# real-world-cryprography/APSU

Measured on AMD Instinct MI355X. Metric: sender query-eval ms (ComputePowers + all BinBundles + gather), 16M-4096 params, lower is better.
Workload: dtype u64; 1 GPU; 16M-4096: n=8192, 4 bundle indices x 7 BinBundles (degrees [1303, 170]), 6 source -> 72 target powers, ps_low_degree=44; db_bytes_rank0=5459379072, binbundles_rank0=28, parallelism=binbundle-shard x1

## Files before the change

apsu_amd/csrc/c_api.cpp:

```cpp
#include "../../include/apsu_he.h"

#include <algorithm>
#include <thread>
#include <atomic>
#include <cstdlib>
#include <cstring>
#include <new>
#include <string>

#include "db_file.h"
#include "engine.h"
#include "multi.h"
#include "wire.h"
#include "seal_codec.h"

using namespace apsu_he;

#include <condition_variable>
#include <mutex>
#include <unordered_set>

struct apsu_he_powers;
struct apsu_he_ctx { std::unique_ptr<Engine> eng; std::unordered_set<apsu_he_powers *> live_powers; int recycling = 0; };
struct apsu_he_relin { std::unique_ptr<RelinKeys> rk; };
// ... 33 lines not shown
        return APSU_HE_OK;
    } catch (const std::invalid_argument &e) { g_last_error = e.what(); return APSU_HE_INVALID_ARGUMENT;
    } catch (const std::logic_error &e) { g_last_error = e.what(); return APSU_HE_LOGIC_ERROR;
    } catch (const std::bad_alloc &e) { g_last_error = e.what(); return APSU_HE_OUT_OF_MEMORY;
    } catch (const HipError &e) {
        g_last_error = e.what();
        if (g_last_error.find("no HIP device") != std::string::npos) return APSU_HE_NO_DEVICE;
        if (g_last_error.find("out of memory") != std::string::npos) return APSU_HE_OUT_OF_MEMORY;
        return APSU_HE_RUNTIME_ERROR;
    } catch (const std::exception &e) { g_last_error = e.what(); return APSU_HE_RUNTIME_ERROR;
    } catch (...) { g_last_error = "unknown error"; return APSU_HE_RUNTIME_ERROR; }
}

#define REQUIRE(cond, msg) do { if (!(cond)) throw std::invalid_argument(msg); } while (0)

extern "C" {

const char *apsu_he_last_error(void) { return g_last_error.c_str(); }
int apsu_he_abi_version(void) { return APSU_HE_ABI_VERSION; }

int apsu_he_create(const char *json, int device, apsu_he_ctx **out)
{
    return guarded([&] {
        REQUIRE(json && out, "null argument");
        PSUParams p = PSUParams::Load(json);
        HeParams hp = HeParams::FromPSUParams(p);
        auto c = new apsu_he_ctx;
        try { c->eng = std::make_unique<Engine>(hp, &p, device); } catch (...) { delete c; throw; }
        *out = c;
    });
}

int apsu_he_create_raw(uint64_t n, const uint64_t *coeff_modulus, int k, uint64_t plain_modulus, int device, apsu_he_ctx **out)
{
    return guarded([&] {
        REQUIRE(coeff_modulus && out && k > 0, "null argument");
        for (int j = 0; j < k; j++) REQUIRE(!(coeff_modulus[j] >> 60), "coeff_modulus prime has more than 60 bits");
        HeParams hp = HeParams::Create((size_t)n, std::vector<u64>(coeff_modulus, coeff_modulus + k), plain_modulus);
        auto c = new apsu_he_ctx;
        try { c->eng = std::make_unique<Engine>(hp, nullptr, device); } catch (...) { delete c; throw; }
        *out = c;
    });
}

int apsu_he_destroy(apsu_he_ctx *ctx)
{
    return guarded([&] {
        if (!ctx) return;
        {
            std::unique_lock<std::mutex> g(g_registry_mu);
            g_registry_cv.wait(g, [&] { return ctx->recycling == 0; });
            for (apsu_he_powers *p : ctx->live_powers) { p->ctx = nullptr; p->p.reset(); }
            ctx->live_powers.clear();
// ... 320 lines not shown
int apsu_he_compute_powers_cost(const apsu_he_ctx *ctx, uint64_t *cost)
{
    return guarded([&] {
        REQUIRE(ctx && cost, "null argument");
        REQUIRE(ctx->eng->psu(), "context was created without PSUParams");
        const PowersDag &dag = ctx->eng->dag();
        *cost = 110u * (uint64_t)(dag.target_powers().size() - dag.source_count());
    });
}

int apsu_he_multi_create(const char *json, const int *devices, int n_devices, apsu_he_multi **out)
{
    return guarded([&] {
        REQUIRE(json && devices && out && n_devices > 0, "null argument");
        PSUParams p = PSUParams::Load(json);
        HeParams hp = HeParams::FromPSUParams(p);
        auto m = new apsu_he_multi;
        try { m->m = std::make_unique<MultiEngine>(hp, p, std::vector<int>(devices, devices + n_devices)); } catch (...) { delete m; throw; }
        *out = m;
    });
}
int apsu_he_multi_destroy(apsu_he_multi *m) { return guarded([&] { delete m; }); }
int apsu_he_multi_device_count(const apsu_he_multi *m, int *n_devices)
{ return guarded([&] { REQUIRE(m && n_devices, "null argument"); *n_devices = m->m->device_count(); }); }
int apsu_he_multi_result_polys(const apsu_he_multi *m, uint32_t *polys)
{ return guarded([&] { REQUIRE(m && polys, "null argument"); *polys = m->m->engine(0).result_polys(); }); }
int apsu_he_multi_relin_upload(apsu_he_multi *m, const uint64_t *ksk)
{ return guarded([&] { REQUIRE(m && ksk, "null argument"); m->m->upload_relin_keys(ksk); }); }
int apsu_he_multi_db_upload_bundle(apsu_he_multi *m, int device_slot, uint32_t bundle_idx, uint32_t cache_idx, uint32_t n_coeffs,
                                   const uint64_t *const *coeff_ptrs, const uint8_t *is_ntt, int *bundle_id)
{
// ... 889 lines not shown
```

apsu_amd/csrc/engine.cpp:

```cpp
#include "engine.h"
#include "sched_policy.h"
#include "seal_codec.h"

#include <algorithm>
#include <array>
#include <cstdlib>
#include <cstring>
#include <stdexcept>

namespace apsu_he {
static uint32_t packed_row_bits(u64 q);

void throw_hip(hipError_t e, const char *file, int line)
{
    throw HipError(std::string("HIP error: ") + hipGetErrorString(e) + " at " + file + ":" + std::to_string(line));
}
#define HIP_CHECK(x) do { hipError_t e_ = (x); if (e_ != hipSuccess) throw_hip(e_, __FILE__, __LINE__); } while (0)

namespace { struct ArenaOverflow { size_t need; }; }

struct Engine::Enter {
    std::lock_guard<std::mutex> lock;
    int prev = -1;
    explicit Enter(Engine *e) : lock(e->mu_)
// ... 104 lines not shown
        }
        d_tabs_.alloc(tabs.size() * sizeof(NttTable));
        HIP_CHECK(hipMemcpy(d_tabs_.p(), tabs.data(), tabs.size() * sizeof(NttTable), hipMemcpyHostToDevice));
        if (const char *v = std::getenv("APSU_HE_SPLIT")) two_stream_default_ = std::atoi(v) != 0 ? 1 : 0;
        if (split_ntt) fuse_tensor_ = false;
        if (const char *v = std::getenv("APSU_HE_MAC_KARA")) mac_kara_ = std::atoi(v) != 0 ? 1 : 0;
        if (const char *v = std::getenv("APSU_HE_EVAL_SIDE")) eval_side_ = std::atoi(v) != 0;
        if (const char *v = std::getenv("APSU_HE_PACKED_ROWS")) packed_rows_ = std::atoi(v) != 0;
        if (!hp_.using_keyswitching) packed_rows_ = false;
        if (const char *v = std::getenv("APSU_HE_EVAL_WS_BYTES")) eval_ws_budget_ = std::strtoull(v, nullptr, 10);
        if (const char *v = std::getenv("APSU_HE_EVAL_PER_TERM")) force_per_term_ = std::atoi(v) != 0;
        if (const char *v = std::getenv("APSU_HE_SEED_EXPAND_HOST")) seed_expand_host_ = std::atoi(v) != 0;
        ntt_latency_limbs_ = NTT_FORM_AUTO;
        data_primes_narrow_ = true;
        for (int j = 0; j < hp_.K; j++) data_primes_narrow_ = data_primes_narrow_ && ntt_is_narrow(hp_.key_q[j], hp_.logn);
        if (const char *v = std::getenv("APSU_HE_FUSE_TAIL")) fuse_tail_ = std::atoi(v) != 0;
        if (const char *v = std::getenv("APSU_HE_NTT_LATENCY_LIMBS")) ntt_latency_limbs_ = std::strtoull(v, nullptr, 10);
    }
    {
        const int nl = hp_.first_chain_idx + 1;
        std::vector<DevLevel> lv(nl);
        std::vector<int> map_ext((size_t)nl * DMAXE, 0), map_ks((size_t)nl * (DMAXL + 1) * DMAXL, 0),
            map_ksacc((size_t)nl * (DMAXL + 1), 0);
        const u64 mt = (u64)1 << 32;
        for (int c = 0; c < nl; c++) {
            const LevelConstants &h = hp_.level[c];
            DevLevel &d = lv[c];
            std::memset(&d, 0, sizeof(d));
            const int L = h.L, nB = h.nB, nBsk = nB + 1;
            if (L > DMAXL || nBsk > DMAXB) throw std::invalid_argument("too many RNS limbs");
// ... 834 lines not shown
    Enter g(this);
    TIER1_SLOTS();
    check_level(chain_idx);
    check_tier1_residues(a, 2, chain_idx, "multiply: operand holds a coefficient outside [0, q)");
    if (b != a) check_tier1_residues(b, 2, chain_idx, "multiply: operand holds a coefficient outside [0, q)");
    const size_t n = hp_.n, L = chain_idx + 1;
    const int E = hlevel(chain_idx).L + hlevel(chain_idx).nB + 1;
    const bool square = (a == b);
    WITH_ARENA({
        const int nop = square ? 1 : 2;
        u64 *in = ws((size_t)nop * 2 * L * n);
        H2D(in, a, 2 * L * n);
        if (!square) H2D(in + 2 * L * n, b, 2 * L * n);
        u64 *ext = ws((size_t)nop * 2 * E * n);
        { PROF(P_BEHZ_EXT, 0); launch_behz_ext(dlevel(chain_idx), hlevel(chain_idx).L, hlevel(chain_idx).nB, in, L * n, 1, ext, n, nop * 2, st_); }
        d_ntt(ext, (size_t)nop * 2 * E, map_ext(chain_idx), E, false, false);
        u64 *d = ws((size_t)3 * E * n), *o = ws(3 * L * n);
        std::vector<TensorJob> tj{ TensorJob{ ext, square ? ext : ext + (size_t)2 * E * n, d } };
        { PROF(P_TENSOR, 0); launch_tensor(dlevel(chain_idx), upload_jobs(tj), n, 1, st_); }
        d_ntt(d, (size_t)3 * E, map_ext_fin(chain_idx), E, true, false);
        std::vector<FinishJob> fj{ FinishJob{ d, o, 1, 0 } };
        { PROF(P_BEHZ_FINISH, 0); launch_behz_finish(dlevel(chain_idx), hlevel(chain_idx).L, hlevel(chain_idx).nB, upload_jobs(fj), false, n, 1, st_); }
        D2H(out3, o, 3 * L * n);
        tier1_done();
    });
}

void Engine::relinearize(u64 *ct3, const RelinKeys &rk, int chain_idx)
{
    Enter g(this);
    TIER1_SLOTS();
    check_level(chain_idx);
    check_tier1_residues(ct3, 3, chain_idx, "relinearize: operand holds a coefficient outside [0, q)");
    if (!hp_.using_keyswitching) throw std::logic_error("parameters do not support key switching");
    const size_t n = hp_.n, L = chain_idx + 1;
// ... 292 lines not shown
                run.dbuf = ws(max_nodes * nb * 3 * Ef * n);
            }
            run.arena_mark = arena_off_;
            return;
        }
        if (stage > 0) {
            if ((size_t)stage >= s.levels.size()) return;
            u64 *dbuf = run.dbuf;
            {
                const size_t d = (size_t)stage;
                arena_off_ = run.arena_mark;
                const auto &pl = s.levels[d - 1];
                const int npar = pl.sp - pl.s0;
                if (npar > 0) {
                    if (run.ext_done != (int)d - 1) { PROFW(P_BEHZ_EXT, (size_t)npar * nb * 2 * n * (Lf + Ef)); launch_behz_ext(dlevel(first), hlevel(first).L, hlevel(first).nB, slot_ptr(pl.s0, 0), slot_w, 2, ext_ptr(pl.s0, 0), n, npar * nb, st_); }
                    d_ntt(ext_ptr(pl.s0, 0), (size_t)npar * nb * 2 * Ef, map_ext(first), (int)Ef, false, false);
                }
                const auto &cl = s.levels[d];
                const int nn = cl.s1 - cl.s0;
                if (nn <= 0) return;
                std::vector<TensorJob> tj;
                std::vector<FinishJob> fj;
                for (auto &nd : s.nodes) {
                    if (nd[0] < cl.s0 || nd[0] >= cl.s1) continue;
                    for (int b = 0; b < nb; b++) {
                        u64 *dd = dbuf + ((size_t)(nd[0] - cl.s0) * nb + b) * 3 * Ef * n;
                        tj.push_back(TensorJob{ ext_ptr(nd[1], b), ext_ptr(nd[2], b), dd });
                        fj.push_back(FinishJob{ dd, slot_ptr(nd[0], b), 1, 0 });
                    }
                }
                if (fuse_tensor_) {
                    PROF(P_NTT_FUSED, tj.size() * 3 * Ef);
                    launch_intt_tensor(hp_.logn, upload_jobs(tj), (int)tj.size(), (int)Ef, Ef * n, nullptr, 0, tabs(), map_ext_fin(first), (int)Ef, st_, ntt_latency_limbs_);
                } else {
                    { PROF(P_TENSOR, 0); launch_tensor(dlevel(first), upload_jobs(tj), n, (int)tj.size(), st_); }
                    d_ntt(dbuf, (size_t)nn * nb * 3 * Ef, map_ext_fin(first), (int)Ef, true, false);
                }
                { PROFW(P_BEHZ_FINISH, fj.size() * 3 * n * (Ef + Lf)); launch_behz_finish(dlevel(first), hlevel(first).L, hlevel(first).nB, upload_jobs(fj), false, n, (int)fj.size(), st_); }
                if (hp_.using_keyswitching && nn > 0) {
                    const int npar_here = ((size_t)d + 1 < s.levels.size()) ? (cl.sp - cl.s0) : 0;
                    if (d_relinearize(slot_ptr(cl.s0, 0), slot_w, nn * nb, *rk, first, npar_here ? ext_ptr(cl.s0, 0) : nullptr, npar_here * nb))
                        run.ext_done = (int)d;
                }
            }
            return;
        }
        arena_off_ = run.arena_mark;
        auto convert = [&](const std::vector<uint32_t> &powers, int target, u64 *out) {
            if (powers.empty()) return;
            const int cnt = (int)powers.size() * nb;
            std::vector<CtJob> jobs;
// ... 28 lines not shown
            for (int b = 0; b < nb; b++)
                for (size_t i = 0; i < np; i++)
                    for (size_t pl = 0; pl < 2 * Lf; pl++)
                        srcp[(((size_t)b * np + i) * 2 * Lf) + pl] = slot_ptr(s.slot_of[s.low_powers[i]], b) + pl * n;
            bool nored = hp_.logn <= 14;
            for (size_t j = 0; j < Lf && nored; j++) nored = ntt_gather_nored_ok(hp_.key_q[j], hp_.key_q[j], hp_.logn);
            PROF(P_NTT_FWD, srcp.size());
            launch_ntt_gather(hp_.logn, upload_jobs(srcp), pw->low.u(), srcp.size(), tabs(), map_ct(), (int)Lf, st_, nored, ntt_latency_limbs_, data_primes_narrow_);
        } else if (do_low) {
            convert(s.low_powers, low_target, pw->low.u());
            d_ntt_ct(pw->low.u(), (size_t)pw->n_low * nb * 2, low_target, false);
        }
        if (do_high && pw->n_high) {
            convert(s.high_powers, high, pw->high.u());
            { PROFW(P_BEHZ_EXT, (size_t)pw->n_high * nb * 2 * n * (Lh + Eh)); launch_behz_ext(dlevel(high), hlevel(high).L, hlevel(high).nB, pw->high.u(), Lh * n, 1, pw->hext.u(), n, (int)(pw->n_high * nb * 2), st_); }
            d_ntt(pw->hext.u(), (size_t)pw->n_high * nb * 2 * Eh, map_ext(high), (int)Eh, false, false);
        }
    }
}

std::unique_ptr<Powers> Engine::compute_powers(const uint32_t *bundle_indices, int nb, const u64 *const *src, bool on_device,
                                               const RelinKeys *rk)
{
    Enter g(this);
    if (!has_psu_) throw std::logic_error("context was created without PSUParams");
    if (nb <= 0) throw std::invalid_argument("no bundle indices given");
    if (hp_.using_keyswitching && dag_.depth() > 0 && !rk) throw std::invalid_argument("relinearization keys are required");
    if (nks_) return compute_powers_nks(bundle_indices, nb, src, on_device);
    const Sched &s = sched_;
    const size_t n = hp_.n;
    job_seq_base_ = 0;
// ... 791 lines not shown
    u64 *ext = ws((size_t)NI * 2 * Eh * n);
    bool fused_drop = false;
    if (low == high + 1) {
        PROFW(P_BEHZ_EXT, (size_t)NI * 2 * n * (Ll + Eh));
        fused_drop = launch_drop_behz_ext(dlevel(high), hlevel(high).L, hlevel(high).nB, inner, Ll * n, 1, ext, n, NI * 2, st_, raw_drop);
    }
    if (!fused_drop) {
        u64 *innerh = inner;
        for (int lv = low; lv > high; lv--) {
            u64 *nxt = ws((size_t)NI * 2 * lv * n);
            { PROFW(P_MODSWITCH, (size_t)NI * 2 * n * (2 * lv + 1)); launch_modswitch(dlevel(lv), innerh, (size_t)2 * (lv + 1) * n, 2, nxt, n, NI, st_); }
            innerh = nxt;
        }
        { PROFW(P_BEHZ_EXT, (size_t)NI * 2 * n * (Lh + Eh)); launch_behz_ext(dlevel(high), hlevel(high).L, hlevel(high).nB, innerh, Lh * n, 1, ext, n, NI * 2, st_); }
    }
    d_ntt(ext, (size_t)NI * 2 * Eh, map_ext(high), (int)Eh, false, false);
    if (async_high) HIP_CHECK(hipStreamWaitEvent(st_, pw.high_ready, 0));
    u64 *result = ws((size_t)Bs * 3 * Lh * n);
    int max_terms = 0;
    for (int x = 0; x < Bs; x++) max_terms = std::max(max_terms, nin[x]);
    u64 q_widest = 0;
    for (size_t j = 0; j < Lh; j++) q_widest = std::max(q_widest, hlevel(high).q[j]);
    const bool summed = !force_per_term_ && Lh <= 4 &&
                        (unsigned __int128)max_terms * q_widest < ((unsigned __int128)1 << 63);
    const size_t w_cf = (size_t)Bs * 2 * Lh * n;
    if (summed) {
        const size_t nBskh = Eh - Lh;
        u64 *dq = ws((size_t)NI * 3 * Lh * n + (size_t)Bs * 3 * nBskh * n + (late_cf ? w_cf : 0));
        u64 *bsum = dq + (size_t)NI * 3 * Lh * n;
        if (late_cf) {
            g.cf = bsum + (size_t)Bs * 3 * nBskh * n;
// ... 46 lines not shown
        std::vector<SumJob> sj;
        for (int x = 0; x < Bs; x++) {
            const int bs = bslot[c0 + g.ids[x]];
            for (int i = 1; i <= nin[x]; i++) {
                const size_t job = (size_t)in_off[x] + i - 1;
                tj.push_back(TensorJob{ ext + job * 2 * Eh * n, hext_ptr(i, bs), dbuf + job * 3 * Eh * n });
                fj.push_back(FinishJob{ dbuf + job * 3 * Eh * n, tbuf + job * 3 * Lh * n, 1, 0 });
            }
            sj.push_back(SumJob{ tbuf + (size_t)in_off[x] * 3 * Lh * n, result + (size_t)x * 3 * Lh * n, nin[x], 0 });
        }
        if (fuse_tensor_ && tj.size() == (size_t)NI) {
            PROF(P_NTT_FUSED, tj.size() * 3 * Eh);
            launch_intt_tensor(hp_.logn, upload_jobs(tj), (int)tj.size(), (int)Eh, Eh * n, nullptr, 0, tabs(), map_ext_fin(high), (int)Eh, st_, ntt_latency_limbs_);
        } else {
            if (!tj.empty()) { PROF(P_TENSOR, 0); launch_tensor(dlevel(high), upload_jobs(tj), n, (int)tj.size(), st_); }
            d_ntt(dbuf, (size_t)NI * 3 * Eh, map_ext_fin(high), (int)Eh, true, false);
        }
        { PROF(P_BEHZ_FINISH, 0); launch_behz_finish(dlevel(high), hlevel(high).L, hlevel(high).nB, upload_jobs(fj), false, n, (int)fj.size(), st_); }
        { PROF(P_BEHZ_FINISH, 0); launch_sum_jobs(dlevel(high), (int)Lh, upload_jobs(sj), 3, n, Bs, st_); }
    }
    u64 *ks_acc = nullptr;
    d_relinearize(result, 3 * Lh * n, Bs, *rk, high, nullptr, 0, fuse_tail_ ? &ks_acc : nullptr);

    u64 *i0 = nullptr;
    if (side && !side_ran) run_side();
    if (side) HIP_CHECK(hipStreamWaitEvent(st_, ev_side_, 0));
    if (side_i0) {
        i0 = i0_side;
    } else if (i0_fast && low == high) {
        i0 = ssum;
    } else if (i0_fast) {
// ... 157 lines not shown
uint32_t Engine::result_size(const Bundle &b) const
{
    if (!has_psu_) throw std::invalid_argument("context has no PSUParams");
    return result_size_for(b.degree);
}

void Engine::d_multiply_sized(const u64 *ea, int sa, const u64 *eb, int sb, u64 *out, int chain_idx)
{
    const size_t n = hp_.n, L = chain_idx + 1;
    const size_t E = hlevel(chain_idx).L + hlevel(chain_idx).nB + 1;
    const int so = sa + sb - 1, so3 = (so + 2) / 3 * 3;
    u64 *d = ws((size_t)so3 * E * n), *o = ws((size_t)so3 * L * n);
    if (so3 > so) HIP_CHECK(hipMemsetAsync(d + (size_t)so * E * n, 0, (size_t)(so3 - so) * E * n * sizeof(u64), st_));
    std::vector<TensorConvJob> tj{ TensorConvJob{ ea, eb, d, sa, sb } };
    { PROF(P_TENSOR, 0); launch_tensor_conv(dlevel(chain_idx), upload_jobs(tj), n, 1, st_); }
    d_ntt(d, (size_t)so3 * E, map_ext_fin(chain_idx), (int)E, true, false);
    std::vector<FinishJob> fj;
    for (int t = 0; t < so3 / 3; t++) fj.push_back(FinishJob{ d + (size_t)3 * t * E * n, o + (size_t)3 * t * L * n, 1, 0 });
    { PROF(P_BEHZ_FINISH, 0); launch_behz_finish(dlevel(chain_idx), hlevel(chain_idx).L, hlevel(chain_idx).nB, upload_jobs(fj), false, n, (int)fj.size(), st_); }
    D2D(out, o, (size_t)so * L * n);
}

void Engine::multiply_sized(const u64 *a, int sa, const u64 *b, int sb, u64 *out, int chain_idx)
{
    Enter g(this);
    TIER1_SLOTS();
    check_level(chain_idx);
    if (sa < 2 || sb < 2 || sa + sb - 1 > (int)CT_SIZE_MAX) throw std::invalid_argument("invalid size");
    check_tier1_residues(a, (size_t)sa, chain_idx, "multiply_sized: operand holds a coefficient outside [0, q)");
    if (b != a) check_tier1_residues(b, (size_t)sb, chain_idx, "multiply_sized: operand holds a coefficient outside [0, q)");
    const size_t n = hp_.n, L = chain_idx + 1;
    const size_t E = hlevel(chain_idx).L + hlevel(chain_idx).nB + 1;
    const bool square = (a == b && sa == sb);
    WITH_ARENA({
        u64 *in = ws((size_t)(sa + (square ? 0 : sb)) * L * n);
        H2D(in, a, (size_t)sa * L * n);
        if (!square) H2D(in + (size_t)sa * L * n, b, (size_t)sb * L * n);
        const int np = sa + (square ? 0 : sb);
        u64 *ext = ws((size_t)np * E * n);
        { PROF(P_BEHZ_EXT, 0); launch_behz_ext(dlevel(chain_idx), hlevel(chain_idx).L, hlevel(chain_idx).nB, in, L * n, 1, ext, n, np, st_); }
        d_ntt(ext, (size_t)np * E, map_ext(chain_idx), (int)E, false, false);
        u64 *o = ws((size_t)(sa + sb - 1) * L * n);
        d_multiply_sized(ext, sa, square ? ext : ext + (size_t)sa * E * n, sb, o, chain_idx);
        D2H(out, o, (size_t)(sa + sb - 1) * L * n);
        sync();
    });
}

std::unique_ptr<Powers> Engine::compute_powers_nks(const uint32_t *bundle_indices, int nb, const u64 *const *src, bool on_device)
{
    if (nks_oversize_)
        throw std::invalid_argument("invalid size: a product of unrelinearized ciphertext powers exceeds SEAL's largest ciphertext");
    const Sched &s = sched_;
    const size_t n = hp_.n, S = nks_S_, P = s.slot_power.size();
    const size_t E = hlevel(0).L + hlevel(0).nB + 1;
    job_seq_base_ = 0;
// ... 29 lines not shown
        std::vector<CtJob> chk;
        for (auto &kv : dag_.nodes()) {
            if (!kv.second.is_source()) continue;
            for (int b = 0; b < nb; b++) {
                const u64 *sp = src[(size_t)b * dag_.source_count() + si];
                if (on_device) D2D(coef_ptr(s.slot_of[kv.first], b), sp, 2 * n);
                else H2D(coef_ptr(s.slot_of[kv.first], b), sp, 2 * n);
                chk.push_back(CtJob{ coef_ptr(s.slot_of[kv.first], b), coef_ptr(s.slot_of[kv.first], b) });
            }
            si++;
        }
        launch_copy_sources(upload_jobs(chk), 2 * n, (int)chk.size(), dlevel(0), 1, n, bad_source_ + query_seq_ % BAD_SLOTS, query_seq_, st_);
        auto extend = [&](int s0, int s1) {
            if (s1 <= s0) return;
            { PROF(P_BEHZ_EXT, 0); launch_behz_ext(dlevel(0), hlevel(0).L, hlevel(0).nB, coef_ptr(s0, 0), S * n, (int)S, ext_ptr(s0, 0), n, (s1 - s0) * nb, st_); }
            d_ntt(ext_ptr(s0, 0), (size_t)(s1 - s0) * nb * S * E, map_ext(0), (int)E, false, false);
        };
        extend(s.levels[0].s0, s.levels[0].s1);
        for (size_t d = 1; d < s.levels.size(); d++) {
            const size_t mark = arena_off_;
            for (const auto &nd : s.nodes) {
                if (nd[0] < s.levels[d].s0 || nd[0] >= s.levels[d].s1) continue;
                const int sa = (int)nks_size_[s.slot_power[nd[1]]], sb = (int)nks_size_[s.slot_power[nd[2]]];
                for (int b = 0; b < nb; b++) {
                    d_multiply_sized(ext_ptr(nd[1], b), sa, ext_ptr(nd[2], b), sb, coef_ptr(nd[0], b), 0);
                    arena_off_ = mark;
                }
            }
            extend(s.levels[d].s0, s.levels[d].s1);
        }
        for (size_t i = 0; i < s.low_powers.size(); i++)
// ... 76 lines not shown
                    cur += (size_t)even(s_in[i]) * n;
                }
                u64 *lowsum = cur, *cf = cur + (size_t)even(s_low) * n;
                low_streams(b.ntt.u(), l, s_low, lowsum);
                for (uint32_t pp = 0; pp < even(s_high) / 2; pp++)
                    ms.push_back(MacStream{ b.lifted.u(), hext_ptr(1, bs) + (size_t)pp * 2 * E * n, cf + (size_t)pp * 2 * n, H, (u32)n,
                                            (u32)(S * E * n), (u32)(E * n), (u32)n, 0, 1 });
                { auto mj = group_mac(ms); PROF(P_MAC, mac_units(mj)); launch_mac(dlevel(0), 1, upload_jobs(mj), n, (int)mj.size(), st_, mac_kara(0, mac_mean_cnt(mj))); }
                d_ntt_ct(blk, (words / n) + even(s_low) + even(s_high), 0, true);
                HIP_CHECK(hipMemsetAsync(result, 0, (size_t)RS * n * sizeof(u64), st_));
                for (uint32_t i = 1; i <= nin; i++) {
                    const size_t mark = arena_off_;
                    const int sa = (int)s_in[i], sb = (int)sz(i * h), so = sa + sb - 1;
                    u64 *iext = ws((size_t)sa * E * n), *prod = ws((size_t)so * n);
                    { PROF(P_BEHZ_EXT, 0); launch_behz_ext(dlevel(0), hlevel(0).L, hlevel(0).nB, inner[i], n, 1, iext, n, sa, st_); }
                    d_ntt(iext, (size_t)sa * E, map_ext(0), (int)E, false, false);
                    d_multiply_sized(iext, sa, hext_ptr(i, bs), sb, prod, 0);
                    { PROF(P_OTHER, 0); launch_add(dlevel(0), result, prod, so, n, 1, st_); }
                    arena_off_ = mark;
                }
                { PROF(P_OTHER, 0); launch_add(dlevel(0), result, lowsum, (int)s_low, n, 1, st_); }
                { PROF(P_OTHER, 0); launch_add(dlevel(0), result, cf, (int)s_high, n, 1, st_); }
            }
            u64 *row = res_ptr(x);
            const u64 *mk = masks_on_device ? masks[x] : mask_d + (size_t)x * n;
            std::vector<EpiJob> ej{ EpiJob{ result, nullptr, nullptr, b.a0.u(), mk, row } };
            { PROF(P_MODSWITCH, 0); launch_eval_epilogue(dlevel(0), 0, upload_jobs(ej), n, hp_.irrelevant_bit_count, n, 1, st_); }
            if (rs[x] > 2) {
                D2D(row + 2 * n, result + 2 * n, (size_t)(rs[x] - 2) * n);
                { PROF(P_OTHER, 0); launch_clear_bits(row + 2 * n, (size_t)(rs[x] - 2) * n, hp_.irrelevant_bit_count, st_); }
            }
// ... 10 lines not shown
```

apsu_amd/csrc/engine.h:

```cpp
#pragma once
#include <hip/hip_runtime.h>

#include <functional>
#include <memory>
#include <mutex>
#include <string>
#include <vector>

#include "device.h"
#include "params.h"
#include "powers_dag.h"

namespace apsu_he {

struct HipError : std::runtime_error { using std::runtime_error::runtime_error; };

class DevBuf {
public:
    DevBuf() = default;
    explicit DevBuf(size_t bytes) { alloc(bytes); }
    ~DevBuf() { release(); }
    DevBuf(const DevBuf &) = delete;
    DevBuf &operator=(const DevBuf &) = delete;
    DevBuf(DevBuf &&o) noexcept : p_(o.p_), bytes_(o.bytes_) { o.p_ = nullptr; o.bytes_ = 0; }
// ... 177 lines not shown
    std::mutex mu_;

    DevBuf d_tabs_, d_tw_, d_levels_, d_key_, d_map_ct_, d_map_ext_, d_map_ext_fin_, d_map_ks_, d_map_ksacc_, d_map_ksacc_raw_, d_fin_, d_drop_, d_mdtw_;
    DevBuf arena_;
    size_t arena_off_ = 0;
    struct Lane { hipStream_t st = nullptr; DevBuf arena; size_t off = 0, job_seq = 0; };
    Lane lanes_[3];
    int cur_lane_ = 0, overflow_lane_ = 0;
    void switch_lane(int lane);
    hipEvent_t ev_main_ = nullptr;
    hipEvent_t ev_fork_ = nullptr, ev_side_ = nullptr, ev_intt_ = nullptr;
    bool inputs_ready_ = false;
    bool pipe_cp_ = true;
    bool force_pipe_ = false;
    bool data_primes_narrow_ = false;
    size_t ntt_latency_limbs_ = 0;
    bool eval_side_ = true;
    bool async_results_ = false;
    std::vector<hipEvent_t> inflight_;
    size_t inflight_head_ = 0, inflight_count_ = 0;
    int max_inflight_ = 2;
    void throttle_inflight();
    void mark_inflight();
    static constexpr int BAD_SLOTS = 16;
    unsigned *bad_source_ = nullptr;
    unsigned bad_reported_[BAD_SLOTS] = {};
    uint32_t query_seq_ = 0;
    void check_sources();
    void check_sources(const Powers &pw);
    bool bad_source_pending(int slot, bool take);
// ... 83 lines not shown
```

apsu_amd/csrc/host_emu.cpp:

```cpp
#define APSU_HOST_EMU 1
#include <cstring>
#include <stdexcept>
#include <string>
#include <vector>

#include "ntt_core.h"
#include "ntt_form.h"
#include "blake2x.h"
#include "params.h"
#include "powers_dag.h"
#include "sched_policy.h"

using namespace apsu_he;

template <int LOGN, int MODE, int PASS, int C = 16> static void emu_pass_tensor(u64 *lds, u64 *glob, int T, const NttTable &tab, const SrcTensor &ops)
{
    if constexpr (PASS < plan_passes(LOGN, C)) {
        if constexpr (PASS == 0)
            for (int tid = 0; tid < T; tid++)
                for (int e = 2 * tid; e < (1 << LOGN); e += 2 * T) *reinterpret_cast<u64x2 *>(lds + lds_slot(e)) = src_load2(ops, glob, e, tab);
        for (int tid = 0; tid < T; tid++) {
            if constexpr (PASS == 0) ntt_pass<LOGN, true, MODE, 0, false, false, SrcTensor, true, TwInline, NoHook, C>(lds, glob, tid, T, tab, ops);
            else ntt_pass<LOGN, true, MODE, PASS, 0, false, SrcPlain, false, TwInline, NoHook, C>(lds, glob, tid, T, tab);
        }
// ... 177 lines not shown
        std::vector<u64> v;
        v.push_back(hp.n); v.push_back(hp.K); v.push_back(hp.first_chain_idx); v.push_back(hp.t);
        for (u64 q : hp.key_q) v.push_back(q);
        for (int j = 0; j < hp.K; j++) v.push_back(hp.ntt[j].psi);
        const LevelConstants &lv = hp.level[hp.first_chain_idx];
        v.push_back(lv.nB); v.push_back(lv.m_sk); v.push_back(lv.gamma);
        for (u64 b : lv.B) v.push_back(b);
        v.push_back(p.bundle_idx_count); v.push_back(p.items_per_bundle); v.push_back(p.item_bit_count);
        v.push_back(hp.irrelevant_bit_count);
        for (size_t i = 0; i < v.size() && (int)i < cap; i++) out[i] = v[i];
        return (int)v.size();
    } catch (const std::invalid_argument &e) { g_err = e.what(); return -1;
    } catch (const std::exception &e) { g_err = e.what(); return -2; }
}

int emu_powers_dag(const uint32_t *sources, int ns, const uint32_t *targets, int nt, uint32_t *nodes)
{
    PowersDag d;
    if (!d.configure(std::set<uint32_t>(sources, sources + ns), std::set<uint32_t>(targets, targets + nt))) return -1;
    int i = 0;
    for (auto &kv : d.nodes()) {
        nodes[4 * i + 0] = kv.second.power; nodes[4 * i + 1] = kv.second.depth;
        nodes[4 * i + 2] = kv.second.parents.first; nodes[4 * i + 3] = kv.second.parents.second;
        i++;
    }
    return (int)d.depth();
}

int emu_create_powers_set(uint32_t ps_low, uint32_t target, uint32_t *out, int cap)
{
// ... 30 lines not shown
```

apsu_amd/csrc/params.cpp:

```cpp
#include "params.h"

#include <algorithm>
#include <cctype>
#include <map>
#include <memory>
#include <stdexcept>

namespace apsu_he {

namespace {

struct JValue {
    enum Kind { Null, Bool, Number, String, Array, Object } kind = Null;
    bool b = false;
    double num = 0;
    bool is_integer = false, negative = false;
    unsigned long long u = 0;
    std::string str;
    std::vector<JValue> arr;
    std::vector<std::pair<std::string, JValue>> obj;

    const JValue *find(const std::string &key) const
    {
        for (auto &kv : obj) if (kv.first == key) return &kv.second;
// ... 384 lines not shown
    }
    u64 divmod(u64 d)
    {
        u128 rem = 0;
        for (size_t i = w.size(); i-- > 0;) { u128 cur = (rem << 64) | w[i]; w[i] = (u64)(cur / d); rem = cur % d; }
        return (u64)rem;
    }
    u64 mod(u64 d) const { Big c = *this; return c.divmod(d); }
    int bits() const
    {
        for (size_t i = w.size(); i-- > 0;) if (w[i]) return (int)(64 * i + 64 - __builtin_clzll(w[i]));
        return 0;
    }
};

LevelConstants make_level(const HeParams &hp, int L)
{
    LevelConstants lv;
    lv.L = L;
    lv.q.assign(hp.key_q.begin(), hp.key_q.begin() + L);
    const u64 t = hp.t;
    Big Q(1);
    for (u64 qj : lv.q) Q.mul(qj);
    int q_bits = Q.bits();
    Big Qt = Q;
    lv.q_mod_t = Qt.divmod(t);
    lv.upper_half_threshold = (t + 1) >> 1;
    for (u64 qj : lv.q) {
        if (qj <= t) throw std::invalid_argument("coeff_modulus primes must exceed plain_modulus (fast plain lift)");
        lv.coeff_div_plain.push_back(Qt.mod(qj));
        lv.upper_half_incr.push_back(qj - t);
    }
    for (int j = 0; j + 1 < L; j++) lv.inv_q_last.push_back(ModulusInfo(lv.q[j]).inv(lv.q[L - 1] % lv.q[j]));

    int t_bits = 64 - __builtin_clzll(t);
    lv.nB = L + ((32 + t_bits + q_bits >= 61 * L + 61) ? 1 : 0);
    if ((size_t)lv.nB + 2 > hp.aux_primes.size()) throw std::logic_error("auxiliary prime list too short");
    lv.m_sk = hp.aux_primes[0];
    lv.gamma = hp.aux_primes[1];
    lv.B.assign(hp.aux_primes.begin() + 2, hp.aux_primes.begin() + 2 + lv.nB);
    std::vector<u64> bsk = lv.B;
    bsk.push_back(lv.m_sk);
    const u64 mt = (u64)1 << 32;

    for (int j = 0; j < L; j++) {
        ModulusInfo mj(lv.q[j]);
        lv.inv_punct_q.push_back(mj.inv(prod_mod(lv.q, j, lv.q[j])));
        lv.q_to_mtilde.push_back(prod_mod(lv.q, j, mt));
    }
    for (u64 m : bsk) {
        std::vector<u64> row;
// ... 14 lines not shown
        lv.inv_punct_B.push_back(ModulusInfo(lv.B[i]).inv(prod_mod(lv.B, i, lv.B[i])));
        lv.B_to_msk.push_back(prod_mod(lv.B, i, lv.m_sk));
    }
    for (int j = 0; j < L; j++) {
        std::vector<u64> row;
        for (int i = 0; i < lv.nB; i++) row.push_back(prod_mod(lv.B, i, lv.q[j]));
        lv.B_to_q.push_back(row);
        lv.prod_B_mod_q.push_back(prod_mod(lv.B, -1, lv.q[j]));
    }
    lv.inv_prod_B_mod_msk = ModulusInfo(lv.m_sk).inv(prod_mod(lv.B, -1, lv.m_sk));
    return lv;
}

}

HeParams HeParams::Create(size_t n, const std::vector<u64> &coeff_modulus, u64 plain_modulus)
{
    HeParams hp;
    if (n < 2 || (n & (n - 1))) throw std::invalid_argument("poly_modulus_degree must be a power of two");
    if (coeff_modulus.empty() || coeff_modulus.size() > (size_t)MAXL) throw std::invalid_argument("coeff_modulus size");
    hp.n = n;
    while (((size_t)1 << hp.logn) < n) hp.logn++;
    hp.K = (int)coeff_modulus.size();
    hp.using_keyswitching = hp.K > 1;
    hp.first_chain_idx = hp.K > 1 ? hp.K - 2 : 0;
    hp.t = plain_modulus;
    hp.key_q = coeff_modulus;
    for (u64 q : hp.key_q)
        if (q >> 61 || (q - 1) % (2 * n) || !is_prime_u64(q)) throw std::invalid_argument("coeff_modulus prime is not NTT-friendly");
    int maxL = hp.first_chain_idx + 1;
    hp.aux_primes = get_primes(2 * (u64)n, 61, (size_t)maxL + 3);
    for (u64 q : hp.key_q) hp.ntt.push_back(make_ntt_tables(q, n, hp.logn));
    for (u64 q : hp.aux_primes) hp.ntt.push_back(make_ntt_tables(q, n, hp.logn));
    if (plain_modulus > 1 && (plain_modulus - 1) % (2 * (u64)n) == 0 && is_prime_u64(plain_modulus)) {
        hp.batching = true;
        hp.ntt.push_back(make_ntt_tables(plain_modulus, n, hp.logn));
        hp.slot_map.resize(n);
        const u64 m = 2 * (u64)n;
        u64 pos = 1;
        const size_t row = n >> 1;
        for (size_t i = 0; i < row; i++) {
            hp.slot_map[i] = bit_reverse((u32)((pos - 1) >> 1), hp.logn);
            hp.slot_map[row | i] = bit_reverse((u32)((m - pos - 1) >> 1), hp.logn);
            pos = (pos * 3) & (m - 1);
        }
    }
    for (int c = 0; c <= hp.first_chain_idx; c++) hp.level.push_back(make_level(hp, c + 1));
    if (hp.K > 1) {
        u64 p = hp.key_q[hp.K - 1];
        for (int j = 0; j < hp.K - 1; j++) hp.inv_p_mod_q.push_back(ModulusInfo(hp.key_q[j]).inv(p % hp.key_q[j]));
    }
    int t_bits = 64 - __builtin_clzll(plain_modulus);
    int q0_bits = 64 - __builtin_clzll(hp.key_q[0]);
    int irr = q0_bits - (t_bits + (hp.logn + 1) - 1);
    hp.irrelevant_bit_count = irr > 0 ? irr : 0;
    return hp;
}

HeParams HeParams::FromPSUParams(const PSUParams &p)
{
    return Create(p.seal_params.poly_modulus_degree,
                  coeff_modulus_create(p.seal_params.poly_modulus_degree, p.seal_params.coeff_modulus_bits),
                  p.seal_params.plain_modulus);
}

}
```

apsu_amd/csrc/params.h:

```cpp
#pragma once
#include <cstdint>
#include <set>
#include <string>
#include <vector>

namespace apsu_he {

typedef uint64_t u64;
typedef unsigned __int128 u128;
typedef uint32_t u32;

struct PSUParams {
    struct TableParams { uint32_t hash_func_count = 0, table_size = 0, max_items_per_bin = 0; } table_params;
    struct ItemParams { uint32_t felts_per_item = 0; } item_params;
    struct QueryParams { uint32_t ps_low_degree = 0; std::set<uint32_t> query_powers; } query_params;
    struct SEALParams {
        size_t poly_modulus_degree = 0;
        std::vector<int> coeff_modulus_bits;
        u64 plain_modulus = 0;
        int plain_modulus_bits = 0;
    } seal_params;

    uint32_t item_bit_count_per_felt = 0, item_bit_count = 0;
    uint32_t items_per_bundle = 0, bins_per_bundle = 0, bundle_idx_count = 0;
// ... 20 lines not shown
std::vector<u64> get_primes(u64 factor, int bit_size, size_t count);
std::vector<u64> coeff_modulus_create(size_t n, const std::vector<int> &bits);
u64 plain_modulus_batching(size_t n, int bits);
u64 minimal_primitive_root(u64 degree, const ModulusInfo &m);

struct NttTablesHost {
    ModulusInfo mod;
    u64 psi = 0;
    std::vector<u64> fwd, fwd_q;
    std::vector<u64> inv, inv_q;
    std::vector<u64> dit, dit_q;
    std::vector<u64> scale, scale_q;
    u64 ninv = 0, ninv_q = 0;
};

constexpr int MAXL = 8;
constexpr int MAXB = MAXL + 2;

struct LevelConstants {
    int L = 0, nB = 0;
    std::vector<u64> q;
    std::vector<u64> B;
    u64 m_sk = 0, gamma = 0;
    std::vector<u64> coeff_div_plain;
    u64 q_mod_t = 0, upper_half_threshold = 0;
    std::vector<u64> upper_half_incr;
    std::vector<u64> inv_q_last;
    std::vector<u64> inv_punct_q;
    std::vector<std::vector<u64>> q_to_bsk;
    std::vector<u64> q_to_mtilde;
// ... 3 lines not shown
    std::vector<std::vector<u64>> B_to_q;
    std::vector<u64> B_to_msk;
    u64 inv_prod_B_mod_msk = 0;
    std::vector<u64> prod_B_mod_q;
};

struct HeParams {
    size_t n = 0;
    int logn = 0;
    int K = 0;
    int first_chain_idx = 0;
    bool using_keyswitching = false;
    u64 t = 0;
    std::vector<u64> key_q;
    std::vector<u64> aux_primes;
    std::vector<NttTablesHost> ntt;
    std::vector<LevelConstants> level;
    std::vector<u64> inv_p_mod_q;
    int irrelevant_bit_count = 0;
    bool batching = false;
    std::vector<uint32_t> slot_map;
    int plain_id() const { return K + (int)aux_primes.size(); }

    static HeParams Create(size_t n, const std::vector<u64> &coeff_modulus, u64 plain_modulus);
    static HeParams FromPSUParams(const PSUParams &p);
    int clamp_chain_idx(int chain_idx) const { return chain_idx > first_chain_idx ? first_chain_idx : chain_idx; }
    int aux_id(int i) const { return K + i; }
    int bsk_id(int level_nB, int i) const { return i < level_nB ? K + 2 + i : K + 0; }
};

}
```

Baseline: 3.269 ms.

## Pick narrow NTT-friendly auxiliary BEHZ primes so extended-base NTTs use narrow path

By default (env APSU_HE_AUX_BASE unset, meaning narrow), the auxiliary BEHZ base primes are chosen by searching for the largest bit size whose primes all satisfy the narrow/lazy NTT conditions. The choice is checked against the SEAL size bound for every level, and the code falls back to the SEAL 61-bit primes if that bound fails. When every extended-base prime is narrow, NTTs over the extended base run in the narrow form instead of the wide one, which is meant to cut the cost of the BEHZ multiply path. The risk is a different auxiliary base than SEAL uses, which could affect correctness margins. It may also require more primes per level if the bound were tight.

```diff
diff --git a/apsu_amd/csrc/c_api.cpp b/apsu_amd/csrc/c_api.cpp
--- a/apsu_amd/csrc/c_api.cpp
+++ b/apsu_amd/csrc/c_api.cpp
@@ -71,6 +71,14 @@
 
 #define REQUIRE(cond, msg) do { if (!(cond)) throw std::invalid_argument(msg); } while (0)
 
+static AuxBase aux_base_from_env()
+{
+    const char *v = std::getenv("APSU_HE_AUX_BASE");
+    if (!v || !*v || !std::strcmp(v, "narrow")) return AuxBase::Narrow;
+    if (!std::strcmp(v, "seal")) return AuxBase::Seal;
+    throw std::invalid_argument("APSU_HE_AUX_BASE must be 'seal' or 'narrow'");
+}
+
 extern "C" {
 
 const char *apsu_he_last_error(void) { return g_last_error.c_str(); }
@@ -81,7 +89,7 @@
     return guarded([&] {
         REQUIRE(json && out, "null argument");
         PSUParams p = PSUParams::Load(json);
-        HeParams hp = HeParams::FromPSUParams(p);
+        HeParams hp = HeParams::FromPSUParams(p, aux_base_from_env());
         auto c = new apsu_he_ctx;
         try { c->eng = std::make_unique<Engine>(hp, &p, device); } catch (...) { delete c; throw; }
         *out = c;
@@ -93,7 +101,7 @@
     return guarded([&] {
         REQUIRE(coeff_modulus && out && k > 0, "null argument");
         for (int j = 0; j < k; j++) REQUIRE(!(coeff_modulus[j] >> 60), "coeff_modulus prime has more than 60 bits");
-        HeParams hp = HeParams::Create((size_t)n, std::vector<u64>(coeff_modulus, coeff_modulus + k), plain_modulus);
+        HeParams hp = HeParams::Create((size_t)n, std::vector<u64>(coeff_modulus, coeff_modulus + k), plain_modulus, aux_base_from_env());
         auto c = new apsu_he_ctx;
         try { c->eng = std::make_unique<Engine>(hp, nullptr, device); } catch (...) { delete c; throw; }
         *out = c;
@@ -444,7 +452,7 @@
     return guarded([&] {
         REQUIRE(json && devices && out && n_devices > 0, "null argument");
         PSUParams p = PSUParams::Load(json);
-        HeParams hp = HeParams::FromPSUParams(p);
+        HeParams hp = HeParams::FromPSUParams(p, aux_base_from_env());
         auto m = new apsu_he_multi;
         try { m->m = std::make_unique<MultiEngine>(hp, p, std::vector<int>(devices, devices + n_devices)); } catch (...) { delete m; throw; }
         *out = m;
diff --git a/apsu_amd/csrc/engine.cpp b/apsu_amd/csrc/engine.cpp
--- a/apsu_amd/csrc/engine.cpp
+++ b/apsu_amd/csrc/engine.cpp
@@ -142,6 +142,8 @@
         ntt_latency_limbs_ = NTT_FORM_AUTO;
         data_primes_narrow_ = true;
         for (int j = 0; j < hp_.K; j++) data_primes_narrow_ = data_primes_narrow_ && ntt_is_narrow(hp_.key_q[j], hp_.logn);
+        ext_primes_narrow_ = data_primes_narrow_;
+        for (u64 m : hp_.aux_primes) ext_primes_narrow_ = ext_primes_narrow_ && ntt_is_narrow(m, hp_.logn);
         if (const char *v = std::getenv("APSU_HE_FUSE_TAIL")) fuse_tail_ = std::atoi(v) != 0;
         if (const char *v = std::getenv("APSU_HE_NTT_LATENCY_LIMBS")) ntt_latency_limbs_ = std::strtoull(v, nullptr, 10);
     }
@@ -1006,11 +1008,11 @@
         if (!square) H2D(in + 2 * L * n, b, 2 * L * n);
         u64 *ext = ws((size_t)nop * 2 * E * n);
         { PROF(P_BEHZ_EXT, 0); launch_behz_ext(dlevel(chain_idx), hlevel(chain_idx).L, hlevel(chain_idx).nB, in, L * n, 1, ext, n, nop * 2, st_); }
-        d_ntt(ext, (size_t)nop * 2 * E, map_ext(chain_idx), E, false, false);
+        d_ntt(ext, (size_t)nop * 2 * E, map_ext(chain_idx), E, false, ext_primes_narrow_);
         u64 *d = ws((size_t)3 * E * n), *o = ws(3 * L * n);
         std::vector<TensorJob> tj{ TensorJob{ ext, square ? ext : ext + (size_t)2 * E * n, d } };
         { PROF(P_TENSOR, 0); launch_tensor(dlevel(chain_idx), upload_jobs(tj), n, 1, st_); }
-        d_ntt(d, (size_t)3 * E, map_ext_fin(chain_idx), E, true, false);
+        d_ntt(d, (size_t)3 * E, map_ext_fin(chain_idx), E, true, ext_primes_narrow_);
         std::vector<FinishJob> fj{ FinishJob{ d, o, 1, 0 } };
         { PROF(P_BEHZ_FINISH, 0); launch_behz_finish(dlevel(chain_idx), hlevel(chain_idx).L, hlevel(chain_idx).nB, upload_jobs(fj), false, n, 1, st_); }
         D2H(out3, o, 3 * L * n);
@@ -1333,7 +1335,7 @@
                 const int npar = pl.sp - pl.s0;
                 if (npar > 0) {
                     if (run.ext_done != (int)d - 1) { PROFW(P_BEHZ_EXT, (size_t)npar * nb * 2 * n * (Lf + Ef)); launch_behz_ext(dlevel(first), hlevel(first).L, hlevel(first).nB, slot_ptr(pl.s0, 0), slot_w, 2, ext_ptr(pl.s0, 0), n, npar * nb, st_); }
-                    d_ntt(ext_ptr(pl.s0, 0), (size_t)npar * nb * 2 * Ef, map_ext(first), (int)Ef, false, false);
+                    d_ntt(ext_ptr(pl.s0, 0), (size_t)npar * nb * 2 * Ef, map_ext(first), (int)Ef, false, ext_primes_narrow_);
                 }
                 const auto &cl = s.levels[d];
                 const int nn = cl.s1 - cl.s0;
@@ -1353,7 +1355,7 @@
                     launch_intt_tensor(hp_.logn, upload_jobs(tj), (int)tj.size(), (int)Ef, Ef * n, nullptr, 0, tabs(), map_ext_fin(first), (int)Ef, st_, ntt_latency_limbs_);
                 } else {
                     { PROF(P_TENSOR, 0); launch_tensor(dlevel(first), upload_jobs(tj), n, (int)tj.size(), st_); }
-                    d_ntt(dbuf, (size_t)nn * nb * 3 * Ef, map_ext_fin(first), (int)Ef, true, false);
+                    d_ntt(dbuf, (size_t)nn * nb * 3 * Ef, map_ext_fin(first), (int)Ef, true, ext_primes_narrow_);
                 }
                 { PROFW(P_BEHZ_FINISH, fj.size() * 3 * n * (Ef + Lf)); launch_behz_finish(dlevel(first), hlevel(first).L, hlevel(first).nB, upload_jobs(fj), false, n, (int)fj.size(), st_); }
                 if (hp_.using_keyswitching && nn > 0) {
@@ -1412,7 +1414,7 @@
         if (do_high && pw->n_high) {
             convert(s.high_powers, high, pw->high.u());
             { PROFW(P_BEHZ_EXT, (size_t)pw->n_high * nb * 2 * n * (Lh + Eh)); launch_behz_ext(dlevel(high), hlevel(high).L, hlevel(high).nB, pw->high.u(), Lh * n, 1, pw->hext.u(), n, (int)(pw->n_high * nb * 2), st_); }
-            d_ntt(pw->hext.u(), (size_t)pw->n_high * nb * 2 * Eh, map_ext(high), (int)Eh, false, false);
+            d_ntt(pw->hext.u(), (size_t)pw->n_high * nb * 2 * Eh, map_ext(high), (int)Eh, false, ext_primes_narrow_);
         }
     }
 }
@@ -2234,7 +2236,7 @@
         }
         { PROFW(P_BEHZ_EXT, (size_t)NI * 2 * n * (Lh + Eh)); launch_behz_ext(dlevel(high), hlevel(high).L, hlevel(high).nB, innerh, Lh * n, 1, ext, n, NI * 2, st_); }
     }
-    d_ntt(ext, (size_t)NI * 2 * Eh, map_ext(high), (int)Eh, false, false);
+    d_ntt(ext, (size_t)NI * 2 * Eh, map_ext(high), (int)Eh, false, ext_primes_narrow_);
     if (async_high) HIP_CHECK(hipStreamWaitEvent(st_, pw.high_ready, 0));
     u64 *result = ws((size_t)Bs * 3 * Lh * n);
     int max_terms = 0;
@@ -2311,7 +2313,7 @@
             launch_intt_tensor(hp_.logn, upload_jobs(tj), (int)tj.size(), (int)Eh, Eh * n, nullptr, 0, tabs(), map_ext_fin(high), (int)Eh, st_, ntt_latency_limbs_);
         } else {
             if (!tj.empty()) { PROF(P_TENSOR, 0); launch_tensor(dlevel(high), upload_jobs(tj), n, (int)tj.size(), st_); }
-            d_ntt(dbuf, (size_t)NI * 3 * Eh, map_ext_fin(high), (int)Eh, true, false);
+            d_ntt(dbuf, (size_t)NI * 3 * Eh, map_ext_fin(high), (int)Eh, true, ext_primes_narrow_);
         }
         { PROF(P_BEHZ_FINISH, 0); launch_behz_finish(dlevel(high), hlevel(high).L, hlevel(high).nB, upload_jobs(fj), false, n, (int)fj.size(), st_); }
         { PROF(P_BEHZ_FINISH, 0); launch_sum_jobs(dlevel(high), (int)Lh, upload_jobs(sj), 3, n, Bs, st_); }
@@ -2499,7 +2501,7 @@
     if (so3 > so) HIP_CHECK(hipMemsetAsync(d + (size_t)so * E * n, 0, (size_t)(so3 - so) * E * n * sizeof(u64), st_));
     std::vector<TensorConvJob> tj{ TensorConvJob{ ea, eb, d, sa, sb } };
     { PROF(P_TENSOR, 0); launch_tensor_conv(dlevel(chain_idx), upload_jobs(tj), n, 1, st_); }
-    d_ntt(d, (size_t)so3 * E, map_ext_fin(chain_idx), (int)E, true, false);
+    d_ntt(d, (size_t)so3 * E, map_ext_fin(chain_idx), (int)E, true, ext_primes_narrow_);
     std::vector<FinishJob> fj;
     for (int t = 0; t < so3 / 3; t++) fj.push_back(FinishJob{ d + (size_t)3 * t * E * n, o + (size_t)3 * t * L * n, 1, 0 });
     { PROF(P_BEHZ_FINISH, 0); launch_behz_finish(dlevel(chain_idx), hlevel(chain_idx).L, hlevel(chain_idx).nB, upload_jobs(fj), false, n, (int)fj.size(), st_); }
@@ -2524,7 +2526,7 @@
         const int np = sa + (square ? 0 : sb);
         u64 *ext = ws((size_t)np * E * n);
         { PROF(P_BEHZ_EXT, 0); launch_behz_ext(dlevel(chain_idx), hlevel(chain_idx).L, hlevel(chain_idx).nB, in, L * n, 1, ext, n, np, st_); }
-        d_ntt(ext, (size_t)np * E, map_ext(chain_idx), (int)E, false, false);
+        d_ntt(ext, (size_t)np * E, map_ext(chain_idx), (int)E, false, ext_primes_narrow_);
         u64 *o = ws((size_t)(sa + sb - 1) * L * n);
         d_multiply_sized(ext, sa, square ? ext : ext + (size_t)sa * E * n, sb, o, chain_idx);
         D2H(out, o, (size_t)(sa + sb - 1) * L * n);
@@ -2584,7 +2586,7 @@
         auto extend = [&](int s0, int s1) {
             if (s1 <= s0) return;
             { PROF(P_BEHZ_EXT, 0); launch_behz_ext(dlevel(0), hlevel(0).L, hlevel(0).nB, coef_ptr(s0, 0), S * n, (int)S, ext_ptr(s0, 0), n, (s1 - s0) * nb, st_); }
-            d_ntt(ext_ptr(s0, 0), (size_t)(s1 - s0) * nb * S * E, map_ext(0), (int)E, false, false);
+            d_ntt(ext_ptr(s0, 0), (size_t)(s1 - s0) * nb * S * E, map_ext(0), (int)E, false, ext_primes_narrow_);
         };
         extend(s.levels[0].s0, s.levels[0].s1);
         for (size_t d = 1; d < s.levels.size(); d++) {
@@ -2691,7 +2693,7 @@
                     const int sa = (int)s_in[i], sb = (int)sz(i * h), so = sa + sb - 1;
                     u64 *iext = ws((size_t)sa * E * n), *prod = ws((size_t)so * n);
                     { PROF(P_BEHZ_EXT, 0); launch_behz_ext(dlevel(0), hlevel(0).L, hlevel(0).nB, inner[i], n, 1, iext, n, sa, st_); }
-                    d_ntt(iext, (size_t)sa * E, map_ext(0), (int)E, false, false);
+                    d_ntt(iext, (size_t)sa * E, map_ext(0), (int)E, false, ext_primes_narrow_);
                     d_multiply_sized(iext, sa, hext_ptr(i, bs), sb, prod, 0);
                     { PROF(P_OTHER, 0); launch_add(dlevel(0), result, prod, so, n, 1, st_); }
                     arena_off_ = mark;
diff --git a/apsu_amd/csrc/engine.h b/apsu_amd/csrc/engine.h
--- a/apsu_amd/csrc/engine.h
+++ b/apsu_amd/csrc/engine.h
@@ -215,6 +215,7 @@
     bool pipe_cp_ = true;
     bool force_pipe_ = false;
     bool data_primes_narrow_ = false;
+    bool ext_primes_narrow_ = false;
     size_t ntt_latency_limbs_ = 0;
     bool eval_side_ = true;
     bool async_results_ = false;
diff --git a/apsu_amd/csrc/host_emu.cpp b/apsu_amd/csrc/host_emu.cpp
--- a/apsu_amd/csrc/host_emu.cpp
+++ b/apsu_amd/csrc/host_emu.cpp
@@ -215,6 +215,23 @@
     } catch (const std::exception &e) { g_err = e.what(); return -2; }
 }
 
+int emu_aux_base(const char *json, int narrow, uint64_t *out, int cap)
+{
+    try {
+        PSUParams p = PSUParams::Load(json);
+        HeParams hp = HeParams::FromPSUParams(p, narrow ? AuxBase::Narrow : AuxBase::Seal);
+        std::vector<u64> v;
+        v.push_back(hp.aux_narrow); v.push_back((u64)hp.aux_bits); v.push_back((u64)hp.logn); v.push_back(hp.level.size());
+        for (const LevelConstants &lv : hp.level) {
+            v.push_back(lv.L); v.push_back(lv.nB); v.push_back(lv.m_sk); v.push_back(lv.gamma);
+            for (u64 b : lv.B) v.push_back(b);
+        }
+        g_err = hp.aux_note;
+        for (size_t i = 0; i < v.size() && (int)i < cap; i++) out[i] = v[i];
+        return (int)v.size();
+    } catch (const std::exception &e) { g_err = e.what(); return -1; }
+}
+
 int emu_powers_dag(const uint32_t *sources, int ns, const uint32_t *targets, int nt, uint32_t *nodes)
 {
     PowersDag d;
diff --git a/apsu_amd/csrc/params.cpp b/apsu_amd/csrc/params.cpp
--- a/apsu_amd/csrc/params.cpp
+++ b/apsu_amd/csrc/params.cpp
@@ -1,4 +1,5 @@
 #include "params.h"
+#include "ntt_core.h"
 
 #include <algorithm>
 #include <cctype>
@@ -422,6 +423,60 @@
     }
 };
 
+int seal_nB(int L, int t_bits, int q_bits) { return L + ((32 + t_bits + q_bits >= 61 * L + 61) ? 1 : 0); }
+
+int prod_bits(const std::vector<u64> &a)
+{
+    Big P(1);
+    for (u64 x : a) P.mul(x);
+    return P.bits();
+}
+
+bool narrow_aux_base(HeParams &hp)
+{
+    const size_t n = hp.n;
+    const int maxL = hp.first_chain_idx + 1;
+    const size_t count = (size_t)maxL + 3;
+    auto usable = [&](u64 q) {
+        NttTable tab{};
+        tab.q = q;
+        tab.narrow = ntt_is_narrow(q, hp.logn) ? 1 : 0;
+        ntt_fold_params(q, tab.fold_k, tab.fold_c);
+        return tab.narrow && ntt_lazy_input_ok(tab, hp.logn);
+    };
+    std::vector<u64> primes;
+    int bits = 0;
+    for (int k = 60; k >= 44 && !bits; k--) {
+        primes.clear();
+        const u64 lower = (u64)1 << (k - 1), f = 2 * (u64)n;
+        bool ok = true;
+        for (u64 v = (((u64)1 << k) - 1) / f * f + 1; primes.size() < count && v > lower && ok; v -= f) {
+            if (!is_prime_u64(v) || v == hp.t || std::find(hp.key_q.begin(), hp.key_q.end(), v) != hp.key_q.end()) continue;
+            ok = usable(v);
+            primes.push_back(v);
+        }
+        if (ok && primes.size() == count) bits = k;
+    }
+    if (!bits) { hp.aux_note = "no bit size gives enough narrow primes with lazy tensor input"; return false; }
+    const int t_bits = 64 - __builtin_clzll(hp.t);
+    for (int L = 1; L <= maxL; L++) {
+        const int q_bits = prod_bits(std::vector<u64>(hp.key_q.begin(), hp.key_q.begin() + L));
+        const int nB = seal_nB(L, t_bits, q_bits);
+        std::vector<u64> bsk(primes.begin() + 2, primes.begin() + 2 + nB);
+        bsk.push_back(primes[0]);
+        const int have = prod_bits(bsk), need = 32 + t_bits + q_bits;
+        if (!(need < have)) {
+            hp.aux_note = "level L = " + std::to_string(L) + ": " + std::to_string(nB + 1) + " primes of " + std::to_string(bits) +
+                          " bits give " + std::to_string(have) + " bits, the size bound needs more than " + std::to_string(need);
+            return false;
+        }
+    }
+    hp.aux_primes = primes;
+    hp.aux_bits = bits;
+    hp.aux_narrow = true;
+    return true;
+}
+
 LevelConstants make_level(const HeParams &hp, int L)
 {
     LevelConstants lv;
@@ -441,8 +496,7 @@
     }
     for (int j = 0; j + 1 < L; j++) lv.inv_q_last.push_back(ModulusInfo(lv.q[j]).inv(lv.q[L - 1] % lv.q[j]));
 
-    int t_bits = 64 - __builtin_clzll(t);
-    lv.nB = L + ((32 + t_bits + q_bits >= 61 * L + 61) ? 1 : 0);
+    lv.nB = seal_nB(L, 64 - __builtin_clzll(t), q_bits);
     if ((size_t)lv.nB + 2 > hp.aux_primes.size()) throw std::logic_error("auxiliary prime list too short");
     lv.m_sk = hp.aux_primes[0];
     lv.gamma = hp.aux_primes[1];
@@ -487,7 +541,7 @@
 
 }
 
-HeParams HeParams::Create(size_t n, const std::vector<u64> &coeff_modulus, u64 plain_modulus)
+HeParams HeParams::Create(size_t n, const std::vector<u64> &coeff_modulus, u64 plain_modulus, AuxBase aux)
 {
     HeParams hp;
     if (n < 2 || (n & (n - 1))) throw std::invalid_argument("poly_modulus_degree must be a power of two");
@@ -503,6 +557,7 @@
         if (q >> 61 || (q - 1) % (2 * n) || !is_prime_u64(q)) throw std::invalid_argument("coeff_modulus prime is not NTT-friendly");
     int maxL = hp.first_chain_idx + 1;
     hp.aux_primes = get_primes(2 * (u64)n, 61, (size_t)maxL + 3);
+    if (aux == AuxBase::Narrow) narrow_aux_base(hp);
     for (u64 q : hp.key_q) hp.ntt.push_back(make_ntt_tables(q, n, hp.logn));
     for (u64 q : hp.aux_primes) hp.ntt.push_back(make_ntt_tables(q, n, hp.logn));
     if (plain_modulus > 1 && (plain_modulus - 1) % (2 * (u64)n) == 0 && is_prime_u64(plain_modulus)) {
@@ -530,11 +585,11 @@
     return hp;
 }
 
-HeParams HeParams::FromPSUParams(const PSUParams &p)
+HeParams HeParams::FromPSUParams(const PSUParams &p, AuxBase aux)
 {
     return Create(p.seal_params.poly_modulus_degree,
                   coeff_modulus_create(p.seal_params.poly_modulus_degree, p.seal_params.coeff_modulus_bits),
-                  p.seal_params.plain_modulus);
-}
-
-}
+                  p.seal_params.plain_modulus, aux);
+}
+
+}
diff --git a/apsu_amd/csrc/params.h b/apsu_amd/csrc/params.h
--- a/apsu_amd/csrc/params.h
+++ b/apsu_amd/csrc/params.h
@@ -58,6 +58,8 @@
     u64 ninv = 0, ninv_q = 0;
 };
 
+enum class AuxBase { Seal, Narrow };
+
 constexpr int MAXL = 8;
 constexpr int MAXB = MAXL + 2;
 
@@ -91,6 +93,9 @@
     u64 t = 0;
     std::vector<u64> key_q;
     std::vector<u64> aux_primes;
+    bool aux_narrow = false;
+    int aux_bits = 61;
+    std::string aux_note;
     std::vector<NttTablesHost> ntt;
     std::vector<LevelConstants> level;
     std::vector<u64> inv_p_mod_q;
@@ -99,8 +104,8 @@
     std::vector<uint32_t> slot_map;
     int plain_id() const { return K + (int)aux_primes.size(); }
 
-    static HeParams Create(size_t n, const std::vector<u64> &coeff_modulus, u64 plain_modulus);
-    static HeParams FromPSUParams(const PSUParams &p);
+    static HeParams Create(size_t n, const std::vector<u64> &coeff_modulus, u64 plain_modulus, AuxBase aux = AuxBase::Seal);
+    static HeParams FromPSUParams(const PSUParams &p, AuxBase aux = AuxBase::Seal);
     int clamp_chain_idx(int chain_idx) const { return chain_idx > first_chain_idx ? first_chain_idx : chain_idx; }
     int aux_id(int i) const { return K + i; }
     int bsk_id(int level_nB, int i) const { return i < level_nB ? K + 2 + i : K + 0; }
```

Result: faster. 3.200 ms, median of 6 (-2.1%).
